# RWails/shadow-1

Measured on AMD Instinct MI355X. Metric: path-table source rows/sec (latency+reliability), higher is better.
Workload: dtype f64; 1 GPU; c4; desc=BA n=100k m=3, 16,384 attached (configs[3], north_star target), vertices=100000, arcs=599982, targets=16384, parallelism=source-row shards x1

## Files before the change

shadow-1_amd/csrc/pe_device.hpp:

```cpp
#pragma once
#include <stdint.h>

namespace shdpe {

struct alignas(16) Arc {
    double lat;
    int32_t col;
    int32_t pad;
};

struct alignas(4) Arc3 {
    int32_t col;
    uint32_t latLo, latHi;
};

struct DevGraph {
    int32_t n;
    int32_t T;
    const int32_t* rowPtr;
    const int32_t* col;
    const double* lat;
    const Arc* arcs;
    const Arc3* arc3;
    const double* rel;
// ... 71 lines not shown
    unsigned char* q = static_cast<unsigned char*>(base);
    for (const TableField& f : TABLE_FIELDS) {
        if (!table_field(wanted, f)) continue;
        set_table_field(v, f, q);
        q += nRows * wanted.T * f.esize;
    }
    return v;
}

struct Tuning {
    int spThreads = 512, heavyDeg = 64, layout = -1, wgPerCU = 8, kflags = 0;
    double deltaFactor = 16.0;
    int exactHc = 0, exactPerCU = 0;
    int batch = -1, batchLB = 0, batchGrid = 0, batchOrder = 2, batchWpe = 0;
    int relabel = 1;
    int batchSplit = 1;
    double batchDeltaFactor = 0.75, batchScratchGB = 64.0;
    double denseMin = 0.25, denseBatchGB = 24.0;
    int densePredMi = 2, denseEpochs = 1;
    int debug = 0, streamWgPerCU = 16;
    int tuneLog = 0;
    int tieCorrupt = 0;
    int pathsGroup = 0;
    int pathsChunk = 0;
    int pathsFast = 1;
    int loadSort = 1;
    int loadSlots = 2048;
    int predFilter = 1;
    int postSplit = -1;
    int laneOffset = 1;
    int failWpe = 0;
    int batchRoundCap = 0;
    int tieSlotsCap = -1;
};

struct DevScratch {
    double* dist;
    int32_t* hops;
    double* rel;
    int32_t* pred;
    double* heapTail;
    int64_t heapStride;
    int32_t* index2;
    int32_t* queue;
    double* lfold;
    int64_t stride;
};

struct alignas(16) BLabel {
    double rel;
    unsigned long long ha;
};

struct BatchScratch {
    unsigned long long* D;
    BLabel* L;
    int32_t* queue;
    int32_t* next;
    int64_t nStride;
    uint32_t* bits;
    int32_t* flags;
    const double* laneOff;
    uint32_t* arcHit;
    int64_t mStride;
    int32_t hitLds;
    unsigned long long* predCnt;
// ... 191 lines not shown
```

shadow-1_amd/csrc/pe_engine.hip:

```cpp
#include <algorithm>
#include <atomic>
#include <cmath>
#include <cstdlib>
#include <cstdio>
#include <cstring>
#include <functional>
#include <memory>
#include <mutex>
#include <new>
#include <chrono>
#include <thread>
#include <vector>

#include "pe_build.hpp"
#include "pe_engine.hpp"
#include "pe_plan.hpp"

using namespace shdpe;

constexpr int LDS_BYTES = 160 * 1024;

template <class T, class A>
static int dev_upload(Shard* s, T** dst, const std::vector<T, A>& src) {
    int rc = dev_alloc(s, dst, src.size());
// ... 16 lines not shown
    if (!(flags & SHD_PE_DEBUG_ENV)) return;
    auto gi = [](const char* k, int& v) { const char* e = std::getenv(k); if (e && *e) v = std::atoi(e); };
    auto gd = [](const char* k, double& v) { const char* e = std::getenv(k); if (e && *e) v = std::atof(e); };
    gi("SHDPE_THREADS", t.spThreads);
    gi("SHDPE_HEAVY_DEG", t.heavyDeg);
    gi("SHDPE_LAYOUT", t.layout);
    gi("SHDPE_WG_PER_CU", t.wgPerCU);
    gi("SHDPE_KFLAGS", t.kflags);
    gd("SHDPE_DELTA_FACTOR", t.deltaFactor);
    gi("SHDPE_EXACT_HC", t.exactHc);
    gi("SHDPE_EXACT_PER_CU", t.exactPerCU);
    gi("SHDPE_BATCH", t.batch);
    gi("SHDPE_BATCH_LB", t.batchLB);
    gi("SHDPE_BATCH_GRID", t.batchGrid);
    gi("SHDPE_BATCH_ORDER", t.batchOrder);
    gi("SHDPE_BATCH_WPE", t.batchWpe);
    gi("SHDPE_RELABEL", t.relabel);
    gi("SHDPE_BATCH_SPLIT", t.batchSplit);
    gd("SHDPE_BATCH_DELTA_FACTOR", t.batchDeltaFactor);
    gd("SHDPE_BATCH_SCRATCH_GB", t.batchScratchGB);
    gd("SHDPE_DENSE_MIN", t.denseMin);
    gd("SHDPE_DENSE_BATCH_GB", t.denseBatchGB);
    gi("SHDPE_PRED_MI", t.densePredMi);
    gi("SHDPE_DENSE_EPOCHS", t.denseEpochs);
    gi("SHDPE_DEBUG", t.debug);
    gi("SHDPE_STREAM_WG_PER_CU", t.streamWgPerCU);
    gi("SHDPE_TIE_CORRUPT", t.tieCorrupt);
    gi("SHDPE_PRED_FILTER", t.predFilter);
    gi("SHDPE_POST_SPLIT", t.postSplit);
    gi("SHDPE_LANE_OFFSET", t.laneOffset);
    gi("SHDPE_TUNE_FAIL_WPE", t.failWpe);
    gi("SHDPE_BATCH_ROUND", t.batchRoundCap);
    gi("SHDPE_TIE_SLOTS", t.tieSlotsCap);
    gi("SHDPE_TUNE_LOG", t.tuneLog);
    gi("SHDPE_PATHS_GROUP", t.pathsGroup);
    gi("SHDPE_PATHS_CHUNK", t.pathsChunk);
    gi("SHDPE_PATHS_FAST", t.pathsFast);
    gi("SHDPE_LOAD_SORT", t.loadSort);
    gi("SHDPE_LOAD_SLOTS", t.loadSlots);
}

extern "C" void shd_pe_default_options(ShdPeOptions* opt) {
    if (!opt) return;
    std::memset(opt, 0, sizeof(*opt));
    opt->device = 0;
    opt->delta = 0.0;
    opt->storePred = 1;
    opt->forceMode = 0;
    opt->nDevices = 1;
    opt->devices = nullptr;
    opt->shardIndex = 0;
    opt->shardCount = 1;
    opt->debugFlags = 0;
}

extern "C" const char* shd_pe_strerror(int code) {
    switch (code) {
        case SHD_PE_OK: return "ok";
        case SHD_PE_EINVAL: return "invalid argument or graph fails topology checks";
        case SHD_PE_ENOMEM: return "out of memory";
        case SHD_PE_ENODEV: return "no usable gfx950 device";
        case SHD_PE_EUNREACHABLE: return "target unreachable";
        case SHD_PE_ENOSELFLOOP: return "self-loop (s,s) missing";
        case SHD_PE_EMULTI: return "multigraph error (reserved: no longer returned)";
        case SHD_PE_EHIP: return "HIP runtime error";
        case SHD_PE_ENOTATTACHED: return "vertex is not attached";
// ... 270 lines not shown
    for (int i = 0; i < o.nDevices; ++i) {
        devs[i] = o.devices ? o.devices[i] : o.device + i;
        if (devs[i] < 0 || devs[i] >= ndev) return SHD_PE_ENODEV;
    }
    return SHD_PE_OK;
}

static double wall_ms(std::chrono::steady_clock::time_point t0) {
    return std::chrono::duration<double, std::milli>(std::chrono::steady_clock::now() - t0).count();
}

static int build_graph_on_device(const ShdPeGraphDesc* graph, const ShdPeOptions& o, const std::vector<int>& devs,
                                 HostGraph* hg, BuiltGraph* built, ShdPeBuildInfo* info) {
    Shard probe;
    probe.device = devs[0];
    int rc = open_device(&probe);
    if (rc) return rc;
    int32_t maxN = BUILD_MAX_N;
    if (o.debugFlags & SHD_PE_DEBUG_ENV) {
        const char* e = std::getenv("SHDPE_BUILD_MAXN");
        if (e && *e && std::atoi(e) > 0) maxN = std::min(maxN, (int32_t)std::atoi(e));
    }
    if ((rc = device_build_graph(graph, devs[0], maxN, hg, built, info))) return rc;
    info->built = info->handedOff ? SHD_PE_BUILD_HOST : SHD_PE_BUILD_DEVICE;
    if (!info->handedOff) return SHD_PE_OK;
    built->release();
    *hg = HostGraph{};
    const auto t0 = std::chrono::steady_clock::now();
    rc = build_host_graph(graph, hg);
    info->msHostBuild = wall_ms(t0);
    return rc;
}

static int create_engine(const ShdPeGraphDesc* graph, const int32_t* attached, int32_t nAttached,
                         const ShdPeOptions* opt, int32_t graphBuild, ShdPeBuildInfo* infoOut, ShdPe** out) {
    if (graphBuild != SHD_PE_BUILD_HOST && graphBuild != SHD_PE_BUILD_DEVICE && graphBuild != SHD_PE_BUILD_AUTO)
        return SHD_PE_EINVAL;
    ShdPeBuildInfo info;
    std::memset(&info, 0, sizeof(info));
    if (infoOut) *infoOut = info;
    if (!out || !graph || nAttached <= 0 || !attached) return SHD_PE_EINVAL;
    *out = nullptr;
    const auto tCreate = std::chrono::steady_clock::now();
    std::unique_ptr<ShdPe> pe(new (std::nothrow) ShdPe());
    if (!pe) return SHD_PE_ENOMEM;
    if (opt) pe->opt = *opt; else shd_pe_default_options(&pe->opt);
    ShdPeOptions& o = pe->opt;
    if (o.nDevices <= 0) o.nDevices = 1;
    if (o.shardCount <= 0) o.shardCount = 1;
    if (o.shardIndex < 0 || o.shardIndex >= o.shardCount || o.nDevices > 64) return SHD_PE_EINVAL;
    read_tuning(pe->tu, o.debugFlags);
    const bool onDevice = graphBuild == SHD_PE_BUILD_DEVICE ||
                          (graphBuild == SHD_PE_BUILD_AUTO && graph->nEdges >= BUILD_AUTO_MIN_EDGES);
    std::vector<int> devs;
    BuiltGraph built;
    int rc;
    if (onDevice) {
        if ((rc = resolve_devices(o, devs))) return rc;
        rc = build_graph_on_device(graph, o, devs, &pe->hg, &built, &info);
    } else {
        const auto t0 = std::chrono::steady_clock::now();
        rc = build_host_graph(graph, &pe->hg);
        info.built = SHD_PE_BUILD_HOST;
        info.msHostBuild = wall_ms(t0);
    }
    if (infoOut) *infoOut = info;
// ... 20 lines not shown
        probe.rowCount = T;
        if ((rc = configure(pe.get(), &probe))) return rc;
    }
    pe->bounds.assign(pe->G + 1, 0);
    (void)shd_pe_plan_shards(T, pe->G, pe->batched ? 16 : 1, pe->bounds.data());
    pe->ownStart = pe->bounds[pe->firstShard];
    pe->ownEnd = pe->bounds[pe->firstShard + o.nDevices];
    Relabelled rl;
    const bool relabel = pe->batched && pe->tu.relabel == 1;
    if (relabel) {
        rl.oldOf = degree_order(g);
        rl.g = relabel_graph(g, rl.oldOf);
        pe->devOf.assign(g.n, 0);
        for (int32_t k = 0; k < g.n; ++k) pe->devOf[rl.oldOf[k]] = k;
        for (int32_t v : pe->attached) rl.attached.push_back(pe->devOf[v]);
    }
    for (int i = 0; i < o.nDevices; ++i) {
        std::unique_ptr<Shard> sh(new (std::nothrow) Shard());
        if (!sh) return SHD_PE_ENOMEM;
        sh->gindex = pe->firstShard + i;
        sh->device = devs[i];
        sh->rowStart = pe->bounds[sh->gindex];
        sh->rowCount = pe->bounds[sh->gindex + 1] - sh->rowStart;
        sh->fullOwner = std::find(devs.begin(), devs.begin() + i, devs[i]) == devs.begin() + i;
        rc = init_shard(pe.get(), sh.get(), relabel ? &rl : nullptr, &built);
        pe->shards.push_back(std::move(sh));
        if (rc) { shd_pe_destroy(pe.release()); return rc; }
    }
    if (pe->mode == 1 && pe->batched) {
        BatchRanks br = batch_ranks(g, pe->attached, pe->posOf, pe->tu.batchOrder);
        pe->rank.swap(br.rank);
        pe->rowOff.swap(br.rowOff);
        pe->hubGroups = std::move(br.groups);
    }
    pe->rowDone.reset(new (std::nothrow) std::atomic<uint8_t>[T]);
    if (!pe->rowDone) { shd_pe_destroy(pe.release()); return SHD_PE_ENOMEM; }
    for (int32_t i = 0; i < T; ++i) pe->rowDone[i].store(0, std::memory_order_relaxed);
    if (infoOut) {
        info.msCreate = wall_ms(tCreate);
        *infoOut = info;
    }
    *out = pe.release();
    return SHD_PE_OK;
}

extern "C" int shd_pe_create(const ShdPeGraphDesc* graph, const int32_t* attached,
                             int32_t nAttached, const ShdPeOptions* opt, ShdPe** out) {
    return create_engine(graph, attached, nAttached, opt, SHD_PE_BUILD_HOST, nullptr, out);
}

extern "C" int shd_pe_create_built(const ShdPeGraphDesc* graph, const int32_t* attached, int32_t nAttached,
                                   const ShdPeOptions* opt, int32_t graphBuild, ShdPeBuildInfo* info,
                                   ShdPe** out) {
    return create_engine(graph, attached, nAttached, opt, graphBuild, info, out);
}

static int digest_dev_graph(Shard* sh, const DevGraph& d, int64_t nArcs, bool withOldId, uint64_t* dAcc,
                            uint64_t* out) {
    const int64_t n = d.n, np1 = d.n + 1;
    struct A { const void* p; int w; int64_t c; };
    const A arr[] = {
        {d.rowPtr, 4, np1}, {d.col, 4, nArcs}, {d.lat, 8, nArcs}, {d.arcs, 8, 2 * nArcs}, {d.arc3, 4, 3 * nArcs},
        {d.rel, 8, nArcs}, {d.inPtr, 4, np1}, {d.inCol, 4, nArcs}, {d.inLat, 8, nArcs}, {d.inRel, 8, nArcs},
        {d.outToIn, 4, nArcs}, {d.vrel, 8, n}, {d.selfLat, 8, n}, {d.selfRel, 8, n}, {d.hasSelf, 1, n},
        {d.selfMinLat, 8, n}, {d.selfMinRel, 8, n}, {d.attached, 4, d.T}, {d.isAttached, 1, n},
        {d.heavyBits, 4, (n + 31) / 32}, {d.flat, 8, nArcs}, {d.srel, 8, nArcs}, {d.oldId, 4, n}};
    const int count = withOldId ? 23 : 22;
    for (int i = 0; i < count; ++i) {
        const int rc = device_array_digest(arr[i].p, arr[i].w, arr[i].c, dAcc, sh->stream, &out[i]);
        if (rc) return rc;
    }
    return SHD_PE_OK;
}

extern "C" int shd_pe_graph_digest(ShdPe* pe, int32_t shard, uint64_t* out, int32_t cap, int32_t* count) {
// ... 134 lines not shown
        release_label_arrays(sh);
        return false;
    }
    sh->postSplitOk = true;
    return true;
}

static int ensure_batch(ShdPe* pe, Shard* sh) {
    if (sh->batchReady) return SHD_PE_OK;
    const size_t NS = ((size_t)pe->hg.n + 63) & ~(size_t)63;
    BatchPlan& plan = sh->plan;
    const size_t LB = (size_t)plan.relax.lb;
    const size_t bitBytes = plan.relax.gbits ? (size_t)batch_bits_words(pe->hg.n) * 4 : 0;
    const size_t perSlot = NS * LB * (8 + 16) + NS * 4 + bitBytes;
    const double budget = pe->tu.batchScratchGB * (double)(1ull << 30);
    const size_t maxSlots = std::max<size_t>(1, (size_t)(budget / (double)perSlot));
    const size_t nBatchesAll = ((size_t)sh->rowCount + LB - 1) / LB;
    size_t grid = 0;
    for (int k = 0; k < plan.nc; ++k) grid = std::max(grid, (size_t)plan.cand[k].grid);
    const size_t slots = std::min<size_t>({grid, maxSlots, std::max<size_t>(1, nBatchesAll)});
    sh->batchSlots = (int32_t)slots;
    for (int k = 0; k < plan.nc; ++k) plan.cand[k].grid = std::min(plan.cand[k].grid, sh->batchSlots);
    plan.relax.grid = std::min(plan.relax.grid, sh->batchSlots);
    plan.post.grid = std::min(plan.post.grid, sh->batchSlots);
    plan.label.grid = std::min(plan.label.grid, sh->batchSlots);
    plan.redo.grid = std::min(plan.redo.grid, sh->batchSlots);
    for (int k = 0; k < plan.nc; ++k) {
        plan.candPred[k].grid = std::min(plan.candPred[k].grid, sh->batchSlots);
        plan.candLabel[k].grid = std::min(plan.candLabel[k].grid, sh->batchSlots);
    }
    int rc;
    const size_t mStride = ((size_t)pe->hg.nArcs() + 127) & ~(size_t)127;
    const bool filter = plan.relax.split && pe->tu.predFilter != 0 && mStride > 0;
    size_t roundB = slots;
    if (plan.relax.split) {
        size_t freeB = 0, totalB = 0;
        if (hipMemGetInfo(&freeB, &totalB) != hipSuccess) freeB = (size_t)16 << 30;
        const size_t perD = NS * LB * 8 + (filter ? mStride / 8 : 0);
        const size_t rest = slots * (perSlot - NS * LB * 8);
        roundB = batch_round_size(slots, nBatchesAll, perD, rest, freeB, pe->tu.batchRoundCap);
    }
    sh->batchRound = (int32_t)roundB;
    if ((rc = dev_alloc(sh, &sh->bsc.D, roundB * NS * LB)) || (rc = dev_alloc(sh, &sh->bsc.L, slots * NS * LB)) ||
        (rc = dev_alloc(sh, &sh->bsc.queue, slots * NS + 16)) ||
        (rc = dev_alloc(sh, &sh->dBatchRows, (size_t)sh->rowsCap + 64)) ||
        (rc = dev_alloc(sh, &sh->dLaneOff, (size_t)sh->rowsCap + 64)) ||
        (rc = dev_alloc(sh, &sh->dBatchAmb, (size_t)sh->rowsCap + 64)) ||
        (rc = dev_alloc(sh, &sh->bsc.flags, roundB + 16)))
        return rc;
    sh->bsc.next = sh->bsc.queue + slots * NS;
    sh->bsc.nStride = (int64_t)NS;
    sh->bsc.arcHit = nullptr;
    sh->bsc.mStride = (int64_t)mStride;
    sh->bsc.hitLds = 0;
    if (filter && dev_alloc(sh, &sh->bsc.arcHit, roundB * (mStride / 32))) (void)hipGetLastError();
    sh->bsc.predCnt = nullptr;
    if (pe->tu.debug && (rc = dev_alloc(sh, &sh->bsc.predCnt, 2))) return rc;
    sh->bsc.LB = nullptr;
    sh->bsc.redo = nullptr;
    sh->bsc.redoRun = 0;
    sh->bsc.bits = nullptr;
    if (bitBytes && (rc = dev_alloc(sh, &sh->bsc.bits, slots * bitBytes / 4))) return rc;
    sh->bsc.laneOff = sh->dLaneOff;
    if ((rc = ensure_tie(pe, sh))) return rc;
    sh->batchReady = true;
    if (plan.postSplit && !ensure_label_arrays(pe, sh)) {
        plan.postSplit = false;
        plan.post = plan.redo;
    }
    return SHD_PE_OK;
}

static int ensure_dense(ShdPe* pe, Shard* sh) {
    if (sh->dW) return SHD_PE_OK;
    const int64_t n = pe->hg.n;
    const int64_t R = std::max<int32_t>(1, sh->rowCount);
    int rc;
    double* w;
    const int64_t budget = (int64_t)(pe->tu.denseBatchGB * (double)(1LL << 30));
    int64_t rows = std::max<int64_t>(64, budget / (n * 12));
    rows = std::min<int64_t>(rows, R);
    if ((rc = dev_alloc(sh, &w, (size_t)(n * n))) || (rc = dev_alloc(sh, &sh->dRl, (size_t)(n * n))) ||
// ... 262 lines not shown
            launch_tie_export(sh->dg, sh->bsc, LB, sh->tie, r0 / sh->batchRound, sh->dBatchAmb + ro,
                              sh->numCUs * 4, pe->tu.tieCorrupt == 3 ? 0 : -1, sh->stream);
        if (roundHook && (rc = (*roundHook)(r0, rn))) return rc;
        if (timed) {
            HIPCHK(hipEventSynchronize(sh->evP[3]));
            trial->msRelax += elapsed(sh->evP[0], sh->evP[1]);
            trial->msPost += elapsed(sh->evP[1], sh->evP[2]);
            trial->msLabel += elapsed(sh->evP[2], sh->evP[3]);
        }
    }
    return SHD_PE_OK;
}

static const BatchLaunch& relax_launch(const Shard* sh, const BatchTrial* trial) {
    return trial ? trial->relax : sh->plan.relax;
}
static PostLaunches post_launches(const Shard* sh, const BatchTrial* trial) {
    if (trial) return PostLaunches{trial->post, trial->label, trial->postSplit ? trial->redo : trial->post,
                                   trial->postSplit};
    const BatchPlan& p = sh->plan;
    return PostLaunches{p.post, p.label, p.redo, p.postSplit};
}

static int relax_batched(ShdPe* pe, Shard* sh, const int32_t* pos, int32_t cnt, ExactWork& x,
                         BatchTrial* trial, const std::vector<int32_t>* batchOrder = nullptr,
                         const RoundHook* roundHook = nullptr) {
    ShdPeStats& st = sh->stats;
    int rc;
    if ((rc = ensure_batch(pe, sh))) return rc;
    const BatchLaunch& relax = relax_launch(sh, trial);
    int32_t nB = 0;
    const int offKind = pe->tu.laneOffset != 0;
    const bool byCost = !batchOrder && !pe->hubGroups.empty();
    std::vector<double> laneOff;
    const std::vector<int32_t> order =
        batchOrder ? *batchOrder
        : byCost ? batch_order_cost(pe->rank, pe->rowOff, pe->hubGroups, pe->hg.meanArcLatency, relax.lb, pos, cnt,
                                    nB, nullptr, &laneOff, offKind)
                 : batch_order(pe->rank, pe->rowOff, relax.lb, pos, cnt, nB);
    if (!byCost) laneOff = lane_offsets(pe->hubGroups, pe->rowOff, order, relax.lb, offKind);
    nB = (int32_t)(order.size() / (size_t)relax.lb);
    HIPCHK(hipMemcpyAsync(sh->dBatchRows, order.data(), order.size() * 4, hipMemcpyHostToDevice, sh->stream));
    HIPCHK(hipMemcpyAsync(sh->dLaneOff, laneOff.data(), laneOff.size() * 8, hipMemcpyHostToDevice, sh->stream));
    if (sh->dDbg) HIPCHK(hipMemsetAsync(sh->dDbg, 0, (size_t)nB * 64, sh->stream));
    if (sh->bsc.predCnt) HIPCHK(hipMemsetAsync(sh->bsc.predCnt, 0, 16, sh->stream));
    if (sh->bsc.redo) HIPCHK(hipMemsetAsync(sh->bsc.redo, 0, 8, sh->stream));
    if (sh->tie.cap > 0) HIPCHK(hipMemsetAsync(sh->tie.count, 0, 4, sh->stream));
    if (sh->tie.req) HIPCHK(hipMemsetAsync(sh->tie.req, 0xFF, (size_t)sh->tie.cap * 16, sh->stream));
    HIPCHK(hipMemsetAsync(sh->bsc.next, 0, 4, sh->stream));
    HIPCHK(hipEventRecord(sh->evA, sh->stream));
    if (!relax.split)
        launch_batch_rows(sh->dg, sh->tab, scratch_at(sh, sh->dBatchRows), sh->dBatchRows, nB, sh->dBatchAmb, relax,
                          sh->dDbg, sh->dTie, sh->stream, 0);
    else if ((rc = batch_rounds(pe, sh, relax, post_launches(sh, trial), nB, trial, roundHook)))
        return rc;
    HIPCHK(hipGetLastError());
    HIPCHK(hipEventRecord(sh->evB, sh->stream));
    std::vector<uint8_t> amb(order.size());
    HIPCHK(hipMemcpyAsync(amb.data(), sh->dBatchAmb, order.size(), hipMemcpyDeviceToHost, sh->stream));
    int32_t redone[2] = {0, 0};
    if (sh->bsc.redo) HIPCHK(hipMemcpyAsync(redone, sh->bsc.redo, 8, hipMemcpyDeviceToHost, sh->stream));
    HIPCHK(hipStreamSynchronize(sh->stream));
    sh->redoBatches += redone[1];
    st.msSparseKernel += elapsed(sh->evA, sh->evB);
    st.launchesSparse++;
    classify_rows(order.data(), order.size(), amb.data(), x);
    if (sh->dDbg) {
        std::vector<int32_t> dbg((size_t)nB * 16);
        HIPCHK(hipMemcpy(dbg.data(), sh->dDbg, dbg.size() * 4, hipMemcpyDeviceToHost));
        print_batch_debug(pe, sh, relax, dbg.data(), nB);
        dump_batches(pe, order, laneOff, dbg, nB, relax.lb);
        if (sh->bsc.predCnt) {
            unsigned long long pc[2] = {0, 0};
            HIPCHK(hipMemcpy(pc, sh->bsc.predCnt, 16, hipMemcpyDeviceToHost));
            sh->predClaimed += (int64_t)pc[0];
            sh->predGathered += (int64_t)pc[1];
            std::fprintf(stderr, "[shdpe] on-demand predecessor pass in-arcs/batch: claimed=%.0f gathered=%.0f "
                         "(%.3f / %.3f x nArcs; filter %s)\n", (double)pc[0] / std::max(nB, 1),
                         (double)pc[1] / std::max(nB, 1), (double)pc[0] / std::max(nB, 1) / (double)pe->hg.nArcs(),
                         (double)pc[1] / std::max(nB, 1) / (double)pe->hg.nArcs(), sh->bsc.arcHit ? "on" : "off");
        }
    }
    return SHD_PE_OK;
}

static int relax_sparse(ShdPe* pe, Shard* sh, const int32_t* pos, int32_t cnt, ExactWork& x) {
    ShdPeStats& st = sh->stats;
    int rc;
    if ((rc = ensure_tie(pe, sh))) return rc;
    if (sh->dTie) HIPCHK(hipMemsetAsync(sh->tie.count, 0, 4, sh->stream));
    HIPCHK(hipEventRecord(sh->evA, sh->stream));
    launch_sparse_rows(sh->dg, sh->tab, sh->sc, sh->dRows, cnt, sh->dRowAmbig, sh->cfg,
                       sh->dDbg, sh->dTie, sh->stream);
    HIPCHK(hipGetLastError());
    HIPCHK(hipEventRecord(sh->evB, sh->stream));
    std::vector<uint8_t> amb(cnt);
    HIPCHK(hipMemcpyAsync(amb.data(), sh->dRowAmbig, cnt, hipMemcpyDeviceToHost, sh->stream));
    HIPCHK(hipStreamSynchronize(sh->stream));
    st.msSparseKernel += elapsed(sh->evA, sh->evB);
    st.launchesSparse++;
    classify_rows(pos, (size_t)cnt, amb.data(), x);
    if (sh->dDbg) {
        std::vector<int32_t> dbg((size_t)cnt * 16);
// ... 1642 lines not shown
```

shadow-1_amd/csrc/pe_engine.hpp:

```cpp
#pragma once
#include <hip/hip_runtime.h>
#include <rccl/rccl.h>

#include <atomic>
#include <memory>
#include <mutex>
#include <vector>

#include "pe_device.hpp"
#include "pe_graph.hpp"
#include "pe_plan.hpp"
#include "shd_pathengine.h"

namespace shdpe {

struct BatchPlan {
    BatchLaunch cand[4];
    BatchLaunch candPred[4], candLabel[4];
    int nc = 0;
    BatchLaunch relax{};
    BatchLaunch post{};
    BatchLaunch label{};
    BatchLaunch redo{};
    bool postSplit = false;
    bool partsOk = false;
    bool tunable() const { return nc > 1; }
};

struct BatchTrial {
    BatchLaunch relax{}, post{}, label{}, redo{};
    bool postSplit = false;
    bool timed = false;
    bool noTable = false;
    double msRelax = 0.0, msPost = 0.0, msLabel = 0.0;
};

struct PathOne {
    int64_t off;
    int32_t len, nFailed;
    PathReq req;
    uint8_t failed, pad[31];
};

struct Shard {
    int gindex = 0;
    int device = 0;
    int numCUs = 256;
    int32_t rowStart = 0, rowCount = 0;
    hipStream_t stream = nullptr;
    hipStream_t copyStream = nullptr;
    hipEvent_t ev0 = nullptr, ev1 = nullptr, evA = nullptr, evB = nullptr;
    hipEvent_t evP[4] = {nullptr, nullptr, nullptr, nullptr};
    std::vector<void*> allocs;
    DevGraph dg{};
    DevGraph dgAux{};
    DevTable tab{};
    DevScratch sc{};
    bool tableReady = false;
    int32_t* dRows = nullptr;
    uint8_t* dRowAmbig = nullptr;
    int32_t* dDbg = nullptr;
    int32_t pathSrc = -1;
    PathOne* dPath = nullptr;
    int32_t rowsCap = 0;
    SparseLaunch cfg{};
    int exactGrid = 0, exactHc = 1;
    BatchPlan plan{};
    int64_t predClaimed = 0, predGathered = 0;
    bool postSplitOk = false;
    int64_t redoBatches = 0;
    bool tuned = false;
    BatchScratch bsc{};
    bool batchReady = false;
    int32_t batchRound = 0;
    int32_t batchSlots = 0;
    int64_t roundsRun = 0, batchesRun = 0;
    int32_t* dBatchRows = nullptr;
    double* dLaneOff = nullptr;
    uint8_t* dBatchAmb = nullptr;
    TieBuf tie{};
    int32_t* dSlots = nullptr;
    TieBuf* dTie = nullptr;
    int32_t* dDenseIdx = nullptr;
    long long* dXdbg = nullptr;
    bool tieTried = false;
    double *dW = nullptr, *dRl = nullptr, *dD = nullptr;
    int32_t* dP = nullptr;
    uint8_t *dRowA = nullptr, *dRowB = nullptr, *dRowAmbD = nullptr, *dChunkEpoch = nullptr;
    unsigned char* dXList = nullptr;
    int32_t* dAny = nullptr;
    int32_t denseRows = 0;
    int32_t* dPosOf = nullptr;
    DevTable full{};
    bool fullOwner = false;
    ncclComm_t comm = nullptr;
    ShdPeStats stats{};
};

}

struct ShdPe {
    shdpe::HostGraph hg;
    std::vector<int32_t> attached;
    std::vector<int32_t> posOf;
    ShdPeOptions opt{};
    shdpe::Tuning tu{};
    int mode = 1;
    bool batched = false;
    std::vector<int32_t> rank;
    std::vector<double> rowOff;
    shdpe::HubGroups hubGroups;
// ... 48 lines not shown
```

shadow-1_amd/csrc/pe_plan.cpp:

```cpp
#include "pe_plan.hpp"

#include <algorithm>
#include <atomic>
#include <climits>
#include <cmath>
#include <functional>
#include <queue>
#include <system_error>
#include <thread>
#include <utility>

namespace shdpe {

std::vector<int32_t> degree_order(const HostGraph& g) {
    std::vector<int32_t> oldOf(g.n);
    for (int32_t v = 0; v < g.n; ++v) oldOf[v] = v;
    std::stable_sort(oldOf.begin(), oldOf.end(), [&](int32_t a, int32_t b) {
        return g.rowPtr[a + 1] - g.rowPtr[a] > g.rowPtr[b + 1] - g.rowPtr[b];
    });
    return oldOf;
}

static std::vector<int32_t> permute_rows(const std::vector<int32_t>& ptr, const std::vector<int32_t>& oldOf,
                                         std::vector<int32_t>& arcNew) {
// ... 249 lines not shown
        if (!nJ) {
            for (int l = 0; l < LB; ++l)
                if (row[l] >= 0 && !rowOff.empty()) off[b0 + l] = rowOff[row[l]];
            continue;
        }
        double mn = INFINITY;
        for (int l = 0; l < LB; ++l)
            if (row[l] >= 0) mn = std::min(mn, S[l]);
        for (int l = 0; l < LB; ++l)
            if (row[l] >= 0) off[b0 + l] = (S[l] - mn) / nJ;
    }
    return off;
}

std::vector<int32_t> batch_order(const std::vector<int32_t>& rank, const std::vector<double>& rowOff,
                                 int LB, const int32_t* pos, int32_t cnt, int32_t& nB) {
    std::vector<int32_t> order = compose_batches(rank, LB, pos, cnt, nB);
    if (!rowOff.empty() && nB > 1) {
        std::vector<std::pair<double, int32_t>> key(nB);
        for (int32_t b = 0; b < nB; ++b) {
            double s = 0.0;
            int c = 0;
            for (int l = 0; l < LB; ++l) {
                const int32_t p = order[(size_t)b * LB + l];
                if (p >= 0) { s += rowOff[p]; ++c; }
            }
            key[b] = {c ? -s / c : 0.0, b};
        }
        sequence_batches(order, LB, key);
    }
    return order;
}

static const double COST_C0 = 0.892, COST_OFF = 0.200, COST_SPREAD = 3.363;

std::vector<int32_t> batch_order_cost(const std::vector<int32_t>& rank, const std::vector<double>& rowOff,
                                      const HubGroups& groups, double meanArcLatency, int LB,
                                      const int32_t* pos, int32_t cnt, int32_t& nB, std::vector<double>* cost,
                                      std::vector<double>* laneOff, int offsetKind) {
    std::vector<int32_t> order = compose_batches(rank, LB, pos, cnt, nB);
    std::vector<double> offs = lane_offsets(groups, rowOff, order, LB, offsetKind);
    const double unit = meanArcLatency > 0.0 && std::isfinite(meanArcLatency) ? meanArcLatency : 1.0;
    const int G = groups.G;
    std::vector<std::pair<double, int32_t>> key(nB);
    std::vector<double> sum(G), sumSq(G);
    std::vector<int> cntOf(G);
    for (int32_t b = 0; b < nB; ++b) {
        std::fill(sum.begin(), sum.end(), 0.0);
        std::fill(sumSq.begin(), sumSq.end(), 0.0);
        std::fill(cntOf.begin(), cntOf.end(), 0);
        double off = 0.0;
        int lanes = 0;
        for (int l = 0; l < LB; ++l) {
            const int32_t p = order[(size_t)b * LB + l];
            if (p < 0) continue;
            ++lanes;
            off += rowOff[p];
            for (int j = 0; j < G; ++j) {
                const double d = groups.dist[(size_t)p * G + j];
                if (!std::isfinite(d)) continue;
                const double x = (d - rowOff[p]) / unit;
                sum[j] += x;
                sumSq[j] += x * x;
                ++cntOf[j];
            }
        }
        double var = 0.0;
// ... 55 lines not shown
```

shadow-1_amd/csrc/pe_plan.hpp:

```cpp
#pragma once
#include <stdint.h>

#include <vector>

#include "pe_graph.hpp"

namespace shdpe {

std::vector<int32_t> degree_order(const HostGraph& g);

HostGraph relabel_graph(const HostGraph& g, const std::vector<int32_t>& oldOf);


constexpr int HUB_GROUPS = 16;

struct HubGroups {
    int G = 0;
    std::vector<double> dist;
    std::vector<int32_t> hub;
    bool empty() const { return G == 0; }
};
HubGroups hub_group_distances(const HostGraph& g, const std::vector<int32_t>& attached, int threads = 0);

struct BatchRanks {
    std::vector<int32_t> rank;
    std::vector<double> rowOff;
    HubGroups groups;
};
BatchRanks batch_ranks(const HostGraph& g, const std::vector<int32_t>& attached,
                       const std::vector<int32_t>& posOf, int order);

std::vector<int32_t> batch_order(const std::vector<int32_t>& rank, const std::vector<double>& rowOff,
                                 int LB, const int32_t* pos, int32_t cnt, int32_t& nB);

std::vector<double> lane_offsets(const HubGroups& groups, const std::vector<double>& rowOff,
                                 const std::vector<int32_t>& order, int LB, int kind = 1);

std::vector<int32_t> batch_order_cost(const std::vector<int32_t>& rank, const std::vector<double>& rowOff,
                                      const HubGroups& groups, double meanArcLatency, int LB,
                                      const int32_t* pos, int32_t cnt, int32_t& nB,
                                      std::vector<double>* cost = nullptr,
                                      std::vector<double>* laneOff = nullptr, int offsetKind = 1);

constexpr size_t ROUND_RESERVE_BYTES = (size_t)12 << 30;
constexpr size_t ROUND_DIST_CAP_BYTES = (size_t)160 << 30;
size_t batch_round_size(size_t slots, size_t nBatchesAll, size_t perD, size_t rest, size_t freeB, int testCap);

int select_mode(const HostGraph& g, int forceMode, double denseMin);

}
```

Measured before the change: 199,300 source rows/s.

## Move cost-based batch planning from host to GPU kernels with rocPRIM sorts

Replaces the host-side batch_order_cost and lane-offset computation with device kernels. They build rank keys, radix-sort the rows, compute per-batch lane offsets and costs with wave shuffles, sort the batches by cost descending, and emit the batch rows and lane offsets. The same emit kernel also folds in the control-buffer resets that used to be separate memsets. The aim is to remove host planning time and the host-to-device copies on the per-call path. In exchange it adds plan scratch memory, which is counted against the round budget, and copies the order back to the host afterwards. Any mismatch with host tie-breaking or floating-point ordering could change batch order.

```diff
diff --git a/shadow-1_amd/csrc/pe_device.hpp b/shadow-1_amd/csrc/pe_device.hpp
--- a/shadow-1_amd/csrc/pe_device.hpp
+++ b/shadow-1_amd/csrc/pe_device.hpp
@@ -127,6 +127,7 @@
     int failWpe = 0;
     int batchRoundCap = 0;
     int tieSlotsCap = -1;
+    int devicePlan = 1;
 };
 
 struct DevScratch {
diff --git a/shadow-1_amd/csrc/pe_engine.hip b/shadow-1_amd/csrc/pe_engine.hip
--- a/shadow-1_amd/csrc/pe_engine.hip
+++ b/shadow-1_amd/csrc/pe_engine.hip
@@ -72,6 +72,7 @@
     gi("SHDPE_TUNE_FAIL_WPE", t.failWpe);
     gi("SHDPE_BATCH_ROUND", t.batchRoundCap);
     gi("SHDPE_TIE_SLOTS", t.tieSlotsCap);
+    gi("SHDPE_DEVICE_PLAN", t.devicePlan);
     gi("SHDPE_TUNE_LOG", t.tuneLog);
     gi("SHDPE_PATHS_GROUP", t.pathsGroup);
     gi("SHDPE_PATHS_CHUNK", t.pathsChunk);
@@ -408,6 +409,8 @@
     return rc;
 }
 
+static int upload_plan_inputs(ShdPe* pe, Shard* sh);
+
 static int create_engine(const ShdPeGraphDesc* graph, const int32_t* attached, int32_t nAttached,
                          const ShdPeOptions* opt, int32_t graphBuild, ShdPeBuildInfo* infoOut, ShdPe** out) {
     if (graphBuild != SHD_PE_BUILD_HOST && graphBuild != SHD_PE_BUILD_DEVICE && graphBuild != SHD_PE_BUILD_AUTO)
@@ -494,6 +497,8 @@
         pe->rank.swap(br.rank);
         pe->rowOff.swap(br.rowOff);
         pe->hubGroups = std::move(br.groups);
+        for (auto& sh : pe->shards)
+            if ((rc = upload_plan_inputs(pe.get(), sh.get()))) { shd_pe_destroy(pe.release()); return rc; }
     }
     pe->rowDone.reset(new (std::nothrow) std::atomic<uint8_t>[T]);
     if (!pe->rowDone) { shd_pe_destroy(pe.release()); return SHD_PE_ENOMEM; }
@@ -503,6 +508,27 @@
         *infoOut = info;
     }
     *out = pe.release();
+    return SHD_PE_OK;
+}
+
+static int upload_plan_inputs(ShdPe* pe, Shard* sh) {
+    const HubGroups& hg = pe->hubGroups;
+    const size_t T = pe->rank.size();
+    if (hg.empty() || hg.G > 64 || T == 0 || pe->rowOff.size() != T || hg.dist.size() != T * (size_t)hg.G)
+        return SHD_PE_OK;
+    HIPCHK(hipSetDevice(sh->device));
+    DevPlan& dp = sh->dplan;
+    int rc;
+    if ((rc = dev_alloc(sh, &dp.rank, T)) || (rc = dev_alloc(sh, &dp.rowOff, T)) ||
+        (rc = dev_alloc(sh, &dp.hubDist, T * (size_t)hg.G)))
+        return rc;
+    HIPCHK(hipMemcpy(dp.rank, pe->rank.data(), T * 4, hipMemcpyHostToDevice));
+    HIPCHK(hipMemcpy(dp.rowOff, pe->rowOff.data(), T * 8, hipMemcpyHostToDevice));
+    HIPCHK(hipMemcpy(dp.hubDist, hg.dist.data(), T * (size_t)hg.G * 8, hipMemcpyHostToDevice));
+    dp.T = (int32_t)T;
+    dp.G = hg.G;
+    const double mean = pe->hg.meanArcLatency;
+    dp.unit = mean > 0.0 && std::isfinite(mean) ? mean : 1.0;
     return SHD_PE_OK;
 }
 
@@ -703,12 +729,20 @@
     int rc;
     const size_t mStride = ((size_t)pe->hg.nArcs() + 127) & ~(size_t)127;
     const bool filter = plan.relax.split && pe->tu.predFilter != 0 && mStride > 0;
+    DevPlan& dp = sh->dplan;
+    size_t planBytes = 0;
+    if (dp.inputs() && pe->tu.devicePlan != 0) {
+        dp.capRows = dp.capBatches = sh->rowsCap;
+        dp.tempBytes = plan_dev_temp_bytes(dp.capRows, dp.capBatches);
+        if (dp.tempBytes)
+            planBytes = dp.tempBytes + ((size_t)dp.capRows + 64) * (12 + 12) + (size_t)dp.capBatches * 24;
+    }
     size_t roundB = slots;
     if (plan.relax.split) {
         size_t freeB = 0, totalB = 0;
         if (hipMemGetInfo(&freeB, &totalB) != hipSuccess) freeB = (size_t)16 << 30;
         const size_t perD = NS * LB * 8 + (filter ? mStride / 8 : 0);
-        const size_t rest = slots * (perSlot - NS * LB * 8);
+        const size_t rest = slots * (perSlot - NS * LB * 8) + planBytes;
         roundB = batch_round_size(slots, nBatchesAll, perD, rest, freeB, pe->tu.batchRoundCap);
     }
     sh->batchRound = (int32_t)roundB;
@@ -719,6 +753,18 @@
         (rc = dev_alloc(sh, &sh->dBatchAmb, (size_t)sh->rowsCap + 64)) ||
         (rc = dev_alloc(sh, &sh->bsc.flags, roundB + 16)))
         return rc;
+    if (planBytes) {
+        const size_t cb = (size_t)dp.capBatches;
+        unsigned char* temp = nullptr;
+        if ((rc = dev_alloc(sh, &dp.keyIn, (size_t)dp.capRows)) || (rc = dev_alloc(sh, &dp.keyOut, (size_t)dp.capRows)) ||
+            (rc = dev_alloc(sh, &dp.sorted, (size_t)dp.capRows)) ||
+            (rc = dev_alloc(sh, &dp.rowsTmp, (size_t)dp.capRows + 64)) ||
+            (rc = dev_alloc(sh, &dp.offTmp, (size_t)dp.capRows + 64)) || (rc = dev_alloc(sh, &dp.cost, cb)) ||
+            (rc = dev_alloc(sh, &dp.costSorted, cb)) || (rc = dev_alloc(sh, &dp.idx, cb)) ||
+            (rc = dev_alloc(sh, &dp.perm, cb)) || (rc = dev_alloc(sh, &temp, dp.tempBytes)))
+            (void)hipGetLastError();
+        dp.temp = rc ? nullptr : temp;
+    }
     sh->bsc.next = sh->bsc.queue + slots * NS;
     sh->bsc.nStride = (int64_t)NS;
     sh->bsc.arcHit = nullptr;
@@ -1047,22 +1093,40 @@
     int32_t nB = 0;
     const int offKind = pe->tu.laneOffset != 0;
     const bool byCost = !batchOrder && !pe->hubGroups.empty();
+    const bool onDevice = byCost && sh->dplan.ready() && pe->tu.devicePlan != 0;
     std::vector<double> laneOff;
-    const std::vector<int32_t> order =
-        batchOrder ? *batchOrder
-        : byCost ? batch_order_cost(pe->rank, pe->rowOff, pe->hubGroups, pe->hg.meanArcLatency, relax.lb, pos, cnt,
-                                    nB, nullptr, &laneOff, offKind)
-                 : batch_order(pe->rank, pe->rowOff, relax.lb, pos, cnt, nB);
-    if (!byCost) laneOff = lane_offsets(pe->hubGroups, pe->rowOff, order, relax.lb, offKind);
-    nB = (int32_t)(order.size() / (size_t)relax.lb);
-    HIPCHK(hipMemcpyAsync(sh->dBatchRows, order.data(), order.size() * 4, hipMemcpyHostToDevice, sh->stream));
-    HIPCHK(hipMemcpyAsync(sh->dLaneOff, laneOff.data(), laneOff.size() * 8, hipMemcpyHostToDevice, sh->stream));
-    if (sh->dDbg) HIPCHK(hipMemsetAsync(sh->dDbg, 0, (size_t)nB * 64, sh->stream));
-    if (sh->bsc.predCnt) HIPCHK(hipMemsetAsync(sh->bsc.predCnt, 0, 16, sh->stream));
-    if (sh->bsc.redo) HIPCHK(hipMemsetAsync(sh->bsc.redo, 0, 8, sh->stream));
-    if (sh->tie.cap > 0) HIPCHK(hipMemsetAsync(sh->tie.count, 0, 4, sh->stream));
-    if (sh->tie.req) HIPCHK(hipMemsetAsync(sh->tie.req, 0xFF, (size_t)sh->tie.cap * 16, sh->stream));
-    HIPCHK(hipMemsetAsync(sh->bsc.next, 0, 4, sh->stream));
+    std::vector<int32_t> order;
+    if (onDevice) {
+        nB = (cnt + relax.lb - 1) / relax.lb;
+        order.resize((size_t)nB * (size_t)relax.lb);
+        PlanControl ctl;
+        ctl.next = sh->bsc.next;
+        ctl.redo = sh->bsc.redo;
+        ctl.predCnt = sh->bsc.predCnt;
+        ctl.tieCount = sh->tie.cap > 0 ? sh->tie.count : nullptr;
+        ctl.tieReq = sh->tie.req;
+        ctl.tieReqWords = sh->tie.req ? (int64_t)sh->tie.cap * 4 : 0;
+        ctl.dbg = sh->dDbg;
+        ctl.dbgWords = sh->dDbg ? (int64_t)nB * 16 : 0;
+        if ((rc = launch_plan_dev(sh->dplan, sh->dRows, cnt, relax.lb, offKind, sh->dBatchRows, sh->dLaneOff, ctl,
+                                  sh->stream)))
+            return rc;
+    } else {
+        order = batchOrder ? *batchOrder
+                : byCost   ? batch_order_cost(pe->rank, pe->rowOff, pe->hubGroups, pe->hg.meanArcLatency, relax.lb,
+                                              pos, cnt, nB, nullptr, &laneOff, offKind)
+                           : batch_order(pe->rank, pe->rowOff, relax.lb, pos, cnt, nB);
+        if (!byCost) laneOff = lane_offsets(pe->hubGroups, pe->rowOff, order, relax.lb, offKind);
+        nB = (int32_t)(order.size() / (size_t)relax.lb);
+        HIPCHK(hipMemcpyAsync(sh->dBatchRows, order.data(), order.size() * 4, hipMemcpyHostToDevice, sh->stream));
+        HIPCHK(hipMemcpyAsync(sh->dLaneOff, laneOff.data(), laneOff.size() * 8, hipMemcpyHostToDevice, sh->stream));
+        if (sh->dDbg) HIPCHK(hipMemsetAsync(sh->dDbg, 0, (size_t)nB * 64, sh->stream));
+        if (sh->bsc.predCnt) HIPCHK(hipMemsetAsync(sh->bsc.predCnt, 0, 16, sh->stream));
+        if (sh->bsc.redo) HIPCHK(hipMemsetAsync(sh->bsc.redo, 0, 8, sh->stream));
+        if (sh->tie.cap > 0) HIPCHK(hipMemsetAsync(sh->tie.count, 0, 4, sh->stream));
+        if (sh->tie.req) HIPCHK(hipMemsetAsync(sh->tie.req, 0xFF, (size_t)sh->tie.cap * 16, sh->stream));
+        HIPCHK(hipMemsetAsync(sh->bsc.next, 0, 4, sh->stream));
+    }
     HIPCHK(hipEventRecord(sh->evA, sh->stream));
     if (!relax.split)
         launch_batch_rows(sh->dg, sh->tab, scratch_at(sh, sh->dBatchRows), sh->dBatchRows, nB, sh->dBatchAmb, relax,
@@ -1073,6 +1137,8 @@
     HIPCHK(hipEventRecord(sh->evB, sh->stream));
     std::vector<uint8_t> amb(order.size());
     HIPCHK(hipMemcpyAsync(amb.data(), sh->dBatchAmb, order.size(), hipMemcpyDeviceToHost, sh->stream));
+    if (onDevice)
+        HIPCHK(hipMemcpyAsync(order.data(), sh->dBatchRows, order.size() * 4, hipMemcpyDeviceToHost, sh->stream));
     int32_t redone[2] = {0, 0};
     if (sh->bsc.redo) HIPCHK(hipMemcpyAsync(redone, sh->bsc.redo, 8, hipMemcpyDeviceToHost, sh->stream));
     HIPCHK(hipStreamSynchronize(sh->stream));
@@ -1084,6 +1150,12 @@
         std::vector<int32_t> dbg((size_t)nB * 16);
         HIPCHK(hipMemcpy(dbg.data(), sh->dDbg, dbg.size() * 4, hipMemcpyDeviceToHost));
         print_batch_debug(pe, sh, relax, dbg.data(), nB);
+        std::fprintf(stderr, "[shdpe] shard %d batch plan by the %s\n", sh->gindex,
+                     onDevice ? "plan kernels" : batchOrder ? "caller" : "host planner");
+        if (onDevice) {
+            laneOff.resize(order.size());
+            HIPCHK(hipMemcpy(laneOff.data(), sh->dLaneOff, laneOff.size() * 8, hipMemcpyDeviceToHost));
+        }
         dump_batches(pe, order, laneOff, dbg, nB, relax.lb);
         if (sh->bsc.predCnt) {
             unsigned long long pc[2] = {0, 0};
diff --git a/shadow-1_amd/csrc/pe_engine.hpp b/shadow-1_amd/csrc/pe_engine.hpp
--- a/shadow-1_amd/csrc/pe_engine.hpp
+++ b/shadow-1_amd/csrc/pe_engine.hpp
@@ -34,6 +34,40 @@
     bool noTable = false;
     double msRelax = 0.0, msPost = 0.0, msLabel = 0.0;
 };
+
+struct DevPlan {
+    int32_t* rank = nullptr;
+    double* rowOff = nullptr;
+    double* hubDist = nullptr;
+    int32_t T = 0, G = 0;
+    double unit = 1.0;
+    uint32_t *keyIn = nullptr, *keyOut = nullptr;
+    int32_t* sorted = nullptr;
+    int32_t* rowsTmp = nullptr;
+    double* offTmp = nullptr;
+    double *cost = nullptr, *costSorted = nullptr;
+    int32_t *idx = nullptr, *perm = nullptr;
+    void* temp = nullptr;
+    size_t tempBytes = 0;
+    int32_t capRows = 0, capBatches = 0;
+    bool inputs() const { return hubDist != nullptr; }
+    bool ready() const { return temp != nullptr; }
+};
+
+struct PlanControl {
+    int32_t* next = nullptr;
+    int32_t* redo = nullptr;
+    unsigned long long* predCnt = nullptr;
+    int32_t* tieCount = nullptr;
+    int32_t* tieReq = nullptr;
+    int64_t tieReqWords = 0;
+    int32_t* dbg = nullptr;
+    int64_t dbgWords = 0;
+};
+
+size_t plan_dev_temp_bytes(int32_t maxRows, int32_t maxBatches);
+int launch_plan_dev(const DevPlan& dp, const int32_t* dPos, int32_t cnt, int32_t LB, int32_t kind,
+                    int32_t* dBatchRows, double* dLaneOff, const PlanControl& ctl, hipStream_t st);
 
 struct PathOne {
     int64_t off;
@@ -77,6 +111,7 @@
     int64_t roundsRun = 0, batchesRun = 0;
     int32_t* dBatchRows = nullptr;
     double* dLaneOff = nullptr;
+    DevPlan dplan{};
     uint8_t* dBatchAmb = nullptr;
     TieBuf tie{};
     int32_t* dSlots = nullptr;
diff --git a/shadow-1_amd/csrc/pe_plan.cpp b/shadow-1_amd/csrc/pe_plan.cpp
--- a/shadow-1_amd/csrc/pe_plan.cpp
+++ b/shadow-1_amd/csrc/pe_plan.cpp
@@ -305,7 +305,6 @@
     return order;
 }
 
-static const double COST_C0 = 0.892, COST_OFF = 0.200, COST_SPREAD = 3.363;
 
 std::vector<int32_t> batch_order_cost(const std::vector<int32_t>& rank, const std::vector<double>& rowOff,
                                       const HubGroups& groups, double meanArcLatency, int LB,
diff --git a/shadow-1_amd/csrc/pe_plan.hpp b/shadow-1_amd/csrc/pe_plan.hpp
--- a/shadow-1_amd/csrc/pe_plan.hpp
+++ b/shadow-1_amd/csrc/pe_plan.hpp
@@ -36,6 +36,7 @@
 std::vector<double> lane_offsets(const HubGroups& groups, const std::vector<double>& rowOff,
                                  const std::vector<int32_t>& order, int LB, int kind = 1);
 
+constexpr double COST_C0 = 0.892, COST_OFF = 0.200, COST_SPREAD = 3.363;
 std::vector<int32_t> batch_order_cost(const std::vector<int32_t>& rank, const std::vector<double>& rowOff,
                                       const HubGroups& groups, double meanArcLatency, int LB,
                                       const int32_t* pos, int32_t cnt, int32_t& nB,
diff --git a/shadow-1_amd/csrc/pe_plan_dev.hip b/shadow-1_amd/csrc/pe_plan_dev.hip
--- /dev/null
+++ b/shadow-1_amd/csrc/pe_plan_dev.hip
@@ -0,0 +1,148 @@
+#include <hip/hip_runtime.h>
+
+#include <algorithm>
+
+#include <rocprim/device/device_radix_sort.hpp>
+
+#include "pe_engine.hpp"
+
+namespace shdpe {
+
+static constexpr int PLAN_THREADS = 256;
+static constexpr int WAVE = 64;
+
+__global__ void k_plan_keys(const int32_t* __restrict__ rank, const int32_t* __restrict__ pos, int32_t cnt,
+                            uint32_t* __restrict__ key) {
+    const int32_t i = blockIdx.x * PLAN_THREADS + threadIdx.x;
+    if (i < cnt) key[i] = (uint32_t)rank[pos[i]];
+}
+
+__device__ static inline double at_least_zero(double v) { return 0.0 < v ? v : 0.0; }
+
+__global__ void k_plan_batch(DevPlan dp, int32_t cnt, int32_t nB, int32_t LB, int32_t kind, double c0, double cOff,
+                             double cSpread) {
+    const int32_t b = blockIdx.x * (PLAN_THREADS / WAVE) + threadIdx.x / WAVE;
+    if (b >= nB) return;
+    const int t = threadIdx.x % WAVE;
+    const int G = dp.G;
+    const int64_t at = (int64_t)b * LB + t;
+    const int32_t p = t < LB && at < cnt ? dp.sorted[at] : -1;
+    const bool real = p >= 0;
+    const double ro = real ? dp.rowOff[p] : 0.0;
+    const double* dist = dp.hubDist + (real ? (int64_t)p * G : 0);
+    double S = 0.0;
+    int nJ = 0;
+    for (int j = 0; kind == 1 && j < G; ++j) {
+        const double d = real ? dist[j] : 0.0;
+        if (!__all(!real || isfinite(d))) continue;
+        ++nJ;
+        if (real) S += d;
+    }
+    double off = ro;
+    if (nJ) {
+        double mn = real ? S : INFINITY;
+        for (int w = WAVE / 2; w > 0; w >>= 1) mn = fmin(mn, __shfl_xor(mn, w));
+        off = (S - mn) / nJ;
+    }
+    if (t < LB) {
+        dp.rowsTmp[at] = p;
+        dp.offTmp[at] = real ? off : 0.0;
+    }
+    double sum = 0.0, sumSq = 0.0, offSum = 0.0;
+    int cntOf = 0, lanes = 0;
+    for (int l = 0; l < LB; ++l) {
+        const int32_t pl = __shfl(p, l);
+        const double rl = __shfl(ro, l);
+        if (pl < 0) continue;
+        ++lanes;
+        offSum += rl;
+        const double d = t < G ? dp.hubDist[(int64_t)pl * G + t] : INFINITY;
+        if (isfinite(d)) {
+            const double x = (d - rl) / dp.unit;
+            sum += x;
+            sumSq += x * x;
+            ++cntOf;
+        }
+    }
+    double var = 0.0;
+    int terms = 0;
+    for (int j = 0; j < G; ++j) {
+        const double sj = __shfl(sum, j), qj = __shfl(sumSq, j);
+        const int cj = __shfl(cntOf, j);
+        if (!cj) continue;
+        var += at_least_zero(qj - sj * sj / cj);
+        terms += cj;
+    }
+    if (t) return;
+    const double spread = terms ? sqrt(var / terms) : 0.0;
+    const double meanOff = lanes ? offSum / lanes / dp.unit : 0.0;
+    dp.cost[b] = (c0 + cOff * meanOff + cSpread * spread) * lanes / LB;
+    dp.idx[b] = b;
+}
+
+__global__ void k_plan_emit(DevPlan dp, int32_t nB, int32_t LB, int32_t* __restrict__ batchRows,
+                            double* __restrict__ laneOff, PlanControl ctl) {
+    const int64_t stride = (int64_t)gridDim.x * PLAN_THREADS;
+    const int64_t t0 = (int64_t)blockIdx.x * PLAN_THREADS + threadIdx.x;
+    for (int64_t i = t0; i < (int64_t)nB * LB; i += stride) {
+        const int64_t from = (int64_t)dp.perm[i / LB] * LB + i % LB;
+        batchRows[i] = dp.rowsTmp[from];
+        laneOff[i] = dp.offTmp[from];
+    }
+    for (int64_t i = t0; i < ctl.tieReqWords; i += stride) ctl.tieReq[i] = -1;
+    for (int64_t i = t0; i < ctl.dbgWords; i += stride) ctl.dbg[i] = 0;
+    if (t0) return;
+    *ctl.next = 0;
+    if (ctl.redo) ctl.redo[0] = ctl.redo[1] = 0;
+    if (ctl.predCnt) ctl.predCnt[0] = ctl.predCnt[1] = 0;
+    if (ctl.tieCount) *ctl.tieCount = 0;
+}
+
+static unsigned bits_of(uint32_t maxValue) {
+    unsigned b = 1;
+    while (b < 32 && (maxValue >> b)) ++b;
+    return b;
+}
+
+size_t plan_dev_temp_bytes(int32_t maxRows, int32_t maxBatches) {
+    size_t a = 0, b = 0;
+    if (rocprim::radix_sort_pairs(nullptr, a, (const uint32_t*)nullptr, (uint32_t*)nullptr, (const int32_t*)nullptr,
+                                  (int32_t*)nullptr, (size_t)maxRows, 0, 32, nullptr) != hipSuccess ||
+        rocprim::radix_sort_pairs_desc(nullptr, b, (const double*)nullptr, (double*)nullptr, (const int32_t*)nullptr,
+                                       (int32_t*)nullptr, (size_t)maxBatches, 0, 64, nullptr) != hipSuccess)
+        return 0;
+    return std::max<size_t>(std::max(a, b), 16);
+}
+
+int launch_plan_dev(const DevPlan& dp, const int32_t* dPos, int32_t cnt, int32_t LB, int32_t kind,
+                    int32_t* dBatchRows, double* dLaneOff, const PlanControl& ctl, hipStream_t st) {
+    if (cnt < 1 || LB < 1 || LB > WAVE || dp.G < 1 || dp.G > WAVE || cnt > dp.capRows) return SHD_PE_EINVAL;
+    const int32_t nB = (cnt + LB - 1) / LB;
+    if (nB > dp.capBatches || (int64_t)nB * LB > (int64_t)dp.capRows + 64) return SHD_PE_EINVAL;
+    hipLaunchKernelGGL(k_plan_keys, dim3((cnt + PLAN_THREADS - 1) / PLAN_THREADS), dim3(PLAN_THREADS), 0, st,
+                       dp.rank, dPos, cnt, dp.keyIn);
+    size_t need = 0, have = dp.tempBytes;
+    const unsigned rankBits = bits_of((uint32_t)std::max(dp.T - 1, 1));
+    if (rocprim::radix_sort_pairs(nullptr, need, dp.keyIn, dp.keyOut, dPos, dp.sorted, (size_t)cnt, 0, rankBits,
+                                  st) != hipSuccess || need > have)
+        return SHD_PE_ENOMEM;
+    if (rocprim::radix_sort_pairs(dp.temp, have, dp.keyIn, dp.keyOut, dPos, dp.sorted, (size_t)cnt, 0, rankBits,
+                                  st) != hipSuccess)
+        return SHD_PE_EHIP;
+    const int perBlock = PLAN_THREADS / WAVE;
+    hipLaunchKernelGGL(k_plan_batch, dim3((nB + perBlock - 1) / perBlock), dim3(PLAN_THREADS), 0, st, dp, cnt, nB,
+                       LB, kind, COST_C0, COST_OFF, COST_SPREAD);
+    have = dp.tempBytes;
+    if (rocprim::radix_sort_pairs_desc(nullptr, need, dp.cost, dp.costSorted, dp.idx, dp.perm, (size_t)nB, 0, 64,
+                                       st) != hipSuccess || need > have)
+        return SHD_PE_ENOMEM;
+    if (rocprim::radix_sort_pairs_desc(dp.temp, have, dp.cost, dp.costSorted, dp.idx, dp.perm, (size_t)nB, 0, 64,
+                                       st) != hipSuccess)
+        return SHD_PE_EHIP;
+    const int64_t work = std::max<int64_t>((int64_t)nB * LB, std::max(ctl.tieReqWords, ctl.dbgWords));
+    const int grid = (int)std::min<int64_t>(1024, (work + PLAN_THREADS - 1) / PLAN_THREADS);
+    hipLaunchKernelGGL(k_plan_emit, dim3(grid), dim3(PLAN_THREADS), 0, st, dp, nB, LB, dBatchRows, dLaneOff, ctl);
+    return hipGetLastError() == hipSuccess ? SHD_PE_OK : SHD_PE_EHIP;
+}
+
+}
```

New measurement: 203,000 source rows/s (median of 6 runs). 1.02x the previous value.
